# dtarb/TauDEM

Hardware: AMD Instinct MI355X
Metric: Mcells/s (PitRemove->D8FlowDir->AreaD8 pipeline) (higher is better)
Workload: dtype f32

## Files before the change

taudem_amd/csrc/flats.hpp:

```cpp
#pragma once
#include <algorithm>
#include <functional>
#include <vector>

#include "context.hpp"
#include "device_common.hpp"
#include "strips.hpp"
#include "tile_relax.hpp"

struct FlatLevels { int T; int Tr; int has_pits; };
struct FlatPhases { const char *classify, *levels, *stats, *directions, *next; };
static inline const FlatPhases& flat_phases(int iteration) {
    static const FlatPhases P[4] = {{"flats 1: classify", "flats 1: level fields", "flats 1: statistics", "flats 1: directions", "flats 1: next elev"},
                                    {"flats 2: classify", "flats 2: level fields", "flats 2: statistics", "flats 2: directions", "flats 2: next elev"},
                                    {"flats 3: classify", "flats 3: level fields", "flats 3: statistics", "flats 3: directions", "flats 3: next elev"},
                                    {"flats 4+: classify", "flats 4+: level fields", "flats 4+: statistics", "flats 4+: directions", "flats 4+: next elev"}};
    return P[iteration < 1 ? 0 : (iteration > 4 ? 3 : iteration - 1)];
}
using lvl_t = int16_t;
constexpr int LVL_SAT = 32767;
constexpr int TDX_FLATS_TOO_DEEP = -4242;
template <class LV>
struct FlatBuffersT { LV* lvl; LV* rq; };
using FlatBuffers = FlatBuffersT<lvl_t>;

template <class LV>
__host__ __device__ __forceinline__ LV flat_elev2(int lvl, int rq, FlatLevels fl) {
    const int e = (lvl < 0) ? 1 : (lvl > 0 ? lvl : 1 + fl.T);
    const int s = (rq > 0) ? (fl.Tr - rq + 1) : 0;
    return (LV)(e + s);
}

namespace flatk {
using namespace tdxk;

constexpr int CLASSIFY_ITEMS = 4;
template <class Traits, class LV>
__global__ __launch_bounds__(256) void classify_kernel(Traits tr, const float* __restrict__ Z, int nx, int tiles_x,
                                                       const uint32_t* __restrict__ list, unsigned long long nq, LV* __restrict__ lvl,
                                                       LV* __restrict__ rq, uint8_t* __restrict__ fmask, uint8_t* __restrict__ rmask,
                                                       uint32_t* __restrict__ tile_flags, uint8_t* __restrict__ tile_masked) {
    const unsigned long long base = (unsigned long long)blockIdx.x * (256 * CLASSIFY_ITEMS) + threadIdx.x;
#pragma unroll
    for (int i = 0; i < CLASSIFY_ITEMS; i++) {
        const unsigned long long q = base + (unsigned long long)i * 256;
        if (q < nq) {
            const size_t c = list[q];
            const float z0 = Z[c];
            bool low = false, quirk = false, higher = false;
            unsigned fm = 0, rm = 0;
#pragma unroll
            for (int k = 1; k <= 8; k++) {
                const size_t n = size_t(ptrdiff_t(c) + ptrdiff_t(d2(k)) * nx + d1(k));
                const float zd = z0 - Z[n];
                const bool inq = lvl[n] >= 0;
                if (zd < 0) higher = true;
                if (inq) rm |= 1u << (k - 1);
                if (!tr.dont_cross(c, nx, k)) {
                    if (zd >= 0 && tr.has_direction(n)) low = true;
                    else if (zd == 0) {
                        if (inq) fm |= 1u << (k - 1);
                        else quirk = true;
                    }
                }
            }
            if (low) lvl[c] = 1;
            else if (quirk) lvl[c] = 2;
            if (higher) rq[c] = 1;
            fmask[c] = uint8_t(low ? 0u : fm);
            rmask[c] = uint8_t(higher ? 0u : rm);
            const unsigned y = unsigned(c / size_t(nx)), x = unsigned(c - size_t(y) * size_t(nx));
            const unsigned tile = (y / tilek::TS) * unsigned(tiles_x) + x / tilek::TS;
            tile_flags[tile] = tilek::FLAG_FULL;
            if (!low && fm != rm) tile_masked[tile] = 1;
        }
    }
}

constexpr int CLS_COLS = 62, CLS_ROWS = 16;
template <class LV, class Src>
__global__ __launch_bounds__(256) void classify_stream_kernel(const float* __restrict__ Z, Src src, int nx, int ny,
                                                                 int y_own0, int y_own1, int tiles_x, LV* __restrict__ lvl,
                                                                 LV* __restrict__ rq, uint8_t* __restrict__ fmask, uint8_t* __restrict__ rmask,
                                                                 uint32_t* __restrict__ tile_flags, uint8_t* __restrict__ tile_masked, int nbx, int xmap,
                                                                 uint8_t* __restrict__ notfull) {
    using tilek::lane_left;
    using tilek::lane_right;
    const int bx = tdxk::xcd_block_x(nbx, xmap);
    if (bx < 0) return;
    const int lx = threadIdx.x & 63;
    const int x = bx * CLS_COLS - 1 + lx;
    const int ybase = __builtin_amdgcn_readfirstlane(y_own0 + blockIdx.y * (4 * CLS_ROWS) + (threadIdx.x >> 6) * CLS_ROWS);
    const bool mine = lx >= 1 && lx <= CLS_COLS && x < nx;
    const bool inx = x >= 0 && x < nx;
    const int xc = x < 0 ? 0 : (x >= nx ? nx - 1 : x);
    float z[CLS_ROWS + 2];
    typename Src::Raw pw[CLS_ROWS + 2];
#pragma unroll
    for (int j = 0; j < CLS_ROWS + 2; j++) {
        const int y = ybase - 1 + j, yc = y < 0 ? 0 : (y >= ny ? ny - 1 : y);
        const size_t o = size_t(yc) * size_t(nx) + size_t(xc);
        z[j] = Z[o];
        pw[j] = src.load(o);
    }
    unsigned ow[CLS_ROWS + 2];
#pragma unroll
    for (int j = 0; j < CLS_ROWS + 2; j++) {
        const int y = ybase - 1 + j;
        const bool in = inx && y >= 0 && y < ny;
        if (!in) z[j] = 0.f;
        ow[j] = in ? Src::onehot(pw[j]) : 0u;
    }
    int flag_row0 = -1, flag_row1 = -1;
    int masked_row = -1;
    unsigned fall_all = 0xFFu, rise_all = 0xFFu;
#pragma unroll
    for (int r = 0; r < CLS_ROWS; r++) {
        const int y = ybase + r;
        const float zn1 = z[r], zc1 = z[r + 1], zs1 = z[r + 2];
        const unsigned on1 = ow[r], oc1 = ow[r + 1], os1 = ow[r + 2];
        const float zn0 = lane_left(zn1, 0.f), zn2 = lane_right(zn1, 0.f), zc0 = lane_left(zc1, 0.f), zc2 = lane_right(zc1, 0.f);
        const float zs0 = lane_left(zs1, 0.f), zs2 = lane_right(zs1, 0.f);
        const unsigned on0 = lane_left(on1, 0u), on2 = lane_right(on1, 0u), oc0 = lane_left(oc1, 0u), oc2 = lane_right(oc1, 0u);
        const unsigned os0 = lane_left(os1, 0u), os2 = lane_right(os1, 0u);
        if (mine && y < y_own1) {
            const size_t idx = size_t(y) * size_t(nx) + size_t(x);
            LV l = -1, q = -1;
            unsigned fm = 0, rm = 0;
            if (oc1 & 1u) {
                const float z0 = zc1;
                bool higher = false;
                unsigned lowi = 0, fmq = 0;
#define TDX_CLS(K, ZN, ON, NC)                                                                                   \
    {                                                                                                             \
        const float zd = z0 - (ZN);                                                                               \
        const unsigned inq = (ON) & 1u, isdir = min((ON) & 0x1FEu, 1u), oth = ((ON) & 0x1FFu) ? 0u : 1u;          \
        higher |= zd < 0;                                                                                         \
        rm |= inq << ((K) - 1);                                                                                   \
        lowi |= zd >= 0 ? ((NC) & isdir) : 0u;                                                                    \
        fmq |= zd == 0 ? ((0u - (NC)) & ((inq << ((K) - 1)) | (oth << 8))) : 0u;                                  \
    }
                TDX_CLS(1, zc2, oc2, 1u)
                TDX_CLS(2, zn2, on2, (((oc2 >> 4) | (on1 >> 8)) & 1u) ^ 1u)
                TDX_CLS(3, zn1, on1, 1u)
                TDX_CLS(4, zn0, on0, (((on1 >> 6) | (oc0 >> 2)) & 1u) ^ 1u)
                TDX_CLS(5, zc0, oc0, 1u)
                TDX_CLS(6, zs0, os0, (((os1 >> 4) | (oc0 >> 8)) & 1u) ^ 1u)
                TDX_CLS(7, zs1, os1, 1u)
                TDX_CLS(8, zs2, os2, (((oc2 >> 6) | (os1 >> 2)) & 1u) ^ 1u)
#undef TDX_CLS
                const bool low = lowi != 0u, quirk = (fmq >> 8) != 0u;
                fm = fmq & 0xFFu;
                l = low ? 1 : (quirk ? 2 : 0);
                q = higher ? 1 : 0;
                const int tr = y / tilek::TS;
                if (!low && fm != rm) masked_row = tr;
                if (low) fm = 0;
                if (higher) rm = 0;
                if (flag_row0 < 0) flag_row0 = tr; else if (tr != flag_row0) flag_row1 = tr;
            }
            lvl[idx] = l;
            rq[idx] = q;
            fmask[idx] = uint8_t(fm);
            rmask[idx] = uint8_t(rm);
            fall_all &= fm;
            rise_all &= rm;
        }
    }
    if (notfull != nullptr && mine) {
        const int ylast = ybase + CLS_ROWS - 1;
        const int tr0 = ybase / tilek::TS, tr1 = (ylast < ny ? ylast : ny - 1) / tilek::TS;
        const bool short_seg = ylast >= y_own1;
        if (fall_all != 0xFFu || short_seg) { notfull[2 * (size_t(tr0) * tiles_x + x / tilek::TS)] = 1; if (tr1 != tr0) notfull[2 * (size_t(tr1) * tiles_x + x / tilek::TS)] = 1; }
        if (rise_all != 0xFFu || short_seg) { notfull[2 * (size_t(tr0) * tiles_x + x / tilek::TS) + 1] = 1; if (tr1 != tr0) notfull[2 * (size_t(tr1) * tiles_x + x / tilek::TS) + 1] = 1; }
    }
    if (flag_row0 >= 0) tile_flags[flag_row0 * tiles_x + x / tilek::TS] = tilek::FLAG_FULL;
    if (flag_row1 >= 0) tile_flags[flag_row1 * tiles_x + x / tilek::TS] = tilek::FLAG_FULL;
    if (masked_row >= 0) {
        tile_masked[flag_row0 * tiles_x + x / tilek::TS] = 1;
        if (flag_row1 >= 0) tile_masked[flag_row1 * tiles_x + x / tilek::TS] = 1;
    }
}

template <class S>
struct LevelPlainT {
    using T = int;
    static constexpr int kUniform = 8;
    S* G;
    const uint8_t* M;
    static __device__ __forceinline__ int inf() { return 0x3fffffff; }
    using Raw = S;
    using CellRaw = uint8_t;
    __device__ __forceinline__ S load_raw(size_t idx) const { return G[idx]; }
    static __device__ __forceinline__ int decode(S g) { return g > 0 ? int(g) : inf(); }
    static __device__ __forceinline__ bool raw_can_move(S g) { return g >= 0; }
    __device__ __forceinline__ void store(size_t idx, int v) const { G[idx] = S(sizeof(S) == 2 && v > LVL_SAT ? LVL_SAT : v); }
    __device__ __forceinline__ uint8_t cell_raw(size_t idx) const { return M[idx]; }
    static __device__ __forceinline__ void cell_decode(uint8_t m, int& lock, unsigned& mask) { lock = m ? 0 : inf(); mask = m; }
    static __device__ __forceinline__ int cell_floor(int lock, int v) { return lock == 0 ? 0 : v; }
    static __device__ __forceinline__ int apply(int lock, int own, int m) { return tilek::med3_raw(m + 1, lock, own); }
    static __device__ __forceinline__ bool settled(int, int v) { return v <= 1; }
    static __device__ __forceinline__ int act_never() { return int(0x80000000u); }
    static __device__ __forceinline__ int act_threshold(uint8_t m, int v) { return m ? v - 1 : act_never(); }
    static __device__ __forceinline__ int act_threshold_raw(S g) { return g >= 0 ? decode(g) - 1 : act_never(); }
};

constexpr int MACRO_KMAX = 8;
constexpr int MACRO_LMAX = MACRO_KMAX * 64 + 2;
constexpr int MACRO_INF = 0x3fffffff;
constexpr int MACRO_LDS_WORDS = 5 * MACRO_LMAX + 4 * (MACRO_LMAX - 2) + 8;

static __global__ __launch_bounds__(64) void find_blocks_kernel(const uint8_t* __restrict__ notfull, int tiles_x, int tiles_y, int nx, int y_lo, int y_hi, int kmax,
                                                                uint32_t* __restrict__ remapF, uint8_t* __restrict__ blkF, uint32_t* __restrict__ remapR, uint8_t* __restrict__ blkR) {
    const int field = int(blockIdx.y);
    uint32_t* const remap = field ? remapR : remapF;
    uint8_t* const blk_k = field ? blkR : blkF;
    const int rx = (tiles_x + 7) / 8;
    const int reg = blockIdx.x * 64 + threadIdx.x;
    if (reg >= rx * ((tiles_y + 7) / 8)) return;
    const int bx0 = (reg % rx) * 8, by0 = (reg / rx) * 8;
    unsigned long long fm = 0;
    const bool vec = (tiles_x & 7) == 0;
    for (int j = 0; j < 8; j++) {
        const int ty = by0 + j;
        if (ty >= tiles_y || ty * tilek::TS < y_lo || (ty + 1) * tilek::TS > y_hi) continue;
        unsigned rowbits = 0;
        if (vec) {
            const uint4 w = *reinterpret_cast<const uint4*>(notfull + 2 * (size_t(ty) * tiles_x + bx0));
            const unsigned ww[4] = {w.x, w.y, w.z, w.w};
#pragma unroll
            for (int i = 0; i < 8; i++) if (((ww[i >> 1] >> (16 * (i & 1) + 8 * field)) & 0xFFu) == 0u) rowbits |= 1u << i;
        } else {
            for (int i = 0; i < 8 && bx0 + i < tiles_x; i++) if (notfull[2 * (size_t(ty) * tiles_x + bx0 + i) + field] == 0) rowbits |= 1u << i;
        }
        for (int i = 0; i < 8; i++) if (bx0 + i >= tiles_x || (bx0 + i + 1) * tilek::TS > nx) rowbits &= ~(1u << i);
        fm |= (unsigned long long)rowbits << (8 * j);
    }
    auto full_block = [&](int i0, int j0, int kk) {
        unsigned long long m = 0;
        for (int b = 0; b < kk; b++) m |= ((kk == 8 ? 0xFFull : (kk == 4 ? 0xFull : 0x3ull)) << i0) << ((j0 + b) * 8);
        return (fm & m) == m;
    };
    for (int j = 0; j < 8; j++) {
        const int ty = by0 + j;
        if (ty >= tiles_y) break;
        for (int i = 0; i < 8; i++) {
            const int tx = bx0 + i;
            if (tx >= tiles_x) break;
            const size_t t = size_t(ty) * tiles_x + tx;
            int k = 0;
            for (int kk = kmax; kk >= 2 && !k; kk >>= 1) if (full_block(i & ~(kk - 1), j & ~(kk - 1), kk)) k = kk;
            if (k) {
                const int i0 = i & ~(k - 1), j0 = j & ~(k - 1);
                remap[t] = uint32_t(size_t(by0 + j0) * tiles_x + bx0 + i0) | (uint32_t(k == 8 ? 3 : (k == 4 ? 2 : 1)) << tilek::TILE_BLK_SHIFT);
                blk_k[t] = uint8_t((i == i0 && j == j0) ? k : 0);
            } else { remap[t] = uint32_t(t); blk_k[t] = 0; }
        }
    }
}

static __global__ __launch_bounds__(256) void block_flags_kernel(uint32_t* __restrict__ flags, const uint32_t* __restrict__ remap, int ntiles) {
    const int t = blockIdx.x * 256 + threadIdx.x;
    if (t < ntiles && tilek::entry_tile(remap[t]) != t) flags[t] = 0u;
}
__device__ __forceinline__ void macro_edge_scans(const int* __restrict__ h, int L, int* __restrict__ pre, int* __restrict__ suf, int* __restrict__ pm, int* __restrict__ sp) {
    const int wv = int(threadIdx.x >> 6), lane = int(threadIdx.x & 63);
    const bool fwd = (wv & 1) == 0;
    int* const out = wv == 0 ? pre : (wv == 1 ? suf : (wv == 2 ? pm : sp));
    int carry = MACRO_INF;
    for (int base = 0; base < L; base += 64) {
        const int j = fwd ? base + lane : L - 1 - base - lane;
        int v = MACRO_INF;
        if (j >= 0 && j < L) { v = h[j]; if (wv == 2) v -= j; else if (wv == 3) v += j; }
        {
#define TDX_MACRO_SCAN_STEP(CTRL, ROWS) { const int t = __builtin_amdgcn_update_dpp(MACRO_INF, v, CTRL, ROWS, 0xf, false); v = t < v ? t : v; }
            TDX_MACRO_SCAN_STEP(0x111, 0xf) TDX_MACRO_SCAN_STEP(0x112, 0xf) TDX_MACRO_SCAN_STEP(0x114, 0xf) TDX_MACRO_SCAN_STEP(0x118, 0xf)
            TDX_MACRO_SCAN_STEP(0x142, 0xa)
            TDX_MACRO_SCAN_STEP(0x143, 0xc)
#undef TDX_MACRO_SCAN_STEP
        }
        v = carry < v ? carry : v;
        if (j >= 0 && j < L) out[j] = v;
        carry = __shfl(v, 63, 64);
    }
}
__device__ __forceinline__ int macro_offer(const int* __restrict__ h, const int* __restrict__ pre, const int* __restrict__ suf, const int* __restrict__ pm,
                                           const int* __restrict__ sp, int L, int a, int d) {
    const int lo = a - d, hi = a + d;
    int near;
    if (lo <= 0) near = pre[hi < L - 1 ? hi : L - 1];
    else if (hi >= L - 1) near = suf[lo];
    else { near = h[lo]; for (int j = lo + 1; j <= hi; j++) near = h[j] < near ? h[j] : near; }
    int best = near + d;
    if (lo - 1 >= 0) { const int f = pm[lo - 1] + a; best = f < best ? f : best; }
    if (hi + 1 <= L - 1) { const int f = sp[hi + 1] - a; best = f < best ? f : best; }
    return best;
}

template <int INC, class S>
struct LevelOpT {
    using T = int;
    static constexpr int kMacroLdsWords = INC == 1 ? MACRO_LDS_WORDS : 0;
    static constexpr int kUniform = 0;
    S* G;
    const uint8_t* M;
    const uint8_t* TM = nullptr;
    static constexpr bool kHasPlain = INC == 1;
    using Plain = LevelPlainT<S>;
    __device__ __forceinline__ Plain plain() const { return Plain{G, M}; }
    __device__ __forceinline__ bool tile_masked(int tile) const { return TM != nullptr && TM[tile] != 0; }
    static __device__ __forceinline__ int inf() { return 0x3fffffff; }
    using Raw = S;
    using CellRaw = uint8_t;
    __device__ __forceinline__ S load_raw(size_t idx) const { return G[idx]; }
    static __device__ __forceinline__ int decode(S g) { return g > 0 ? int(g) : inf(); }
    static __device__ __forceinline__ bool raw_can_move(S g) { return g >= 0; }
    __device__ __forceinline__ void store(size_t idx, int v) const { G[idx] = S(v); }
    __device__ __forceinline__ uint8_t cell_raw(size_t idx) const { return M[idx]; }
    static __device__ __forceinline__ void cell_decode(uint8_t m, int& cst, unsigned& mask) { cst = 0; mask = m; }
    static __device__ __forceinline__ int apply(int, int own, int m) {
        int t = m + INC;
        if (sizeof(S) == 2 && INC) t = unsigned(t - LVL_SAT) < unsigned(inf() - LVL_SAT) ? LVL_SAT : t;
        return t < own ? t : own;
    }
    static __device__ __forceinline__ int cell_floor(int cst, int) { return cst; }
    static __device__ __forceinline__ bool settled(int, int v) { return v <= 1; }
    static __device__ __forceinline__ int act_never() { return int(0x80000000u); }
    static __device__ __forceinline__ int act_threshold(uint8_t m, int v) { return m ? v - INC : act_never(); }
    static __device__ __forceinline__ int act_threshold_raw(S g) { return g >= 0 ? decode(g) - INC : act_never(); }

    __device__ __forceinline__ int macro_update(const tilek::TileGeom& g, int tile, int k, int* __restrict__ lds, tilek::TileLds& TL, uint32_t* __restrict__ flags_next,
                                                unsigned long long* __restrict__ dbg = nullptr) const {
        const int tid = int(threadIdx.x);
        const unsigned long long tq0 = dbg ? __builtin_readcyclecounter() : 0ull;
        const int W = k * tilek::TS, L = W + 2;
        const int tx0 = tile % g.tiles_x, ty0 = tile / g.tiles_x;
        const int X0 = tx0 * tilek::TS, Y0 = ty0 * tilek::TS;
        const size_t pitch = size_t(g.nx);
        int* const h = lds; int* const pre = h + MACRO_LMAX; int* const suf = pre + MACRO_LMAX; int* const pm = suf + MACRO_LMAX; int* const sp = pm + MACRO_LMAX;
        int* const acc = sp + MACRO_LMAX;
        int* const moved = acc + 4 * (MACRO_LMAX - 2);
        constexpr int AW = MACRO_LMAX - 2;
        if (tid < 8) moved[tid] = 0;
        __syncthreads();
        auto rim_idx = [&](int e, int i) -> size_t {
            const int x = e == 2 ? 0 : (e == 3 ? W - 1 : i), y = e == 0 ? 0 : (e == 1 ? W - 1 : i);
            return size_t(Y0 + y) * pitch + size_t(X0 + x);
        };
        S raw_rim[4][2], raw_ring[4][3];
        unsigned ring_ok = 0;
        int out_target = -1;
        if (tid < 4 * (k + 2)) {
            const int e = tid / (k + 2), j = tid % (k + 2) - 1;
            const int ntx = e == 2 ? tx0 - 1 : (e == 3 ? tx0 + k : tx0 + j), nty = e == 0 ? ty0 - 1 : (e == 1 ? ty0 + k : ty0 + j);
            if (ntx >= 0 && ntx < g.tiles_x && nty >= 0 && nty < g.tiles_y) out_target = int(g.remap[size_t(nty) * g.tiles_x + ntx]);
        }
#pragma unroll
        for (int e = 0; e < 4; e++)
#pragma unroll
            for (int u = 0; u < 2; u++) {
                const int i = tid + u * 256;
                raw_rim[e][u] = G[rim_idx(e, i < W ? i : W - 1)];
// ... 410 lines not shown
    if (nq_old) hipLaunchKernelGGL((flatk::unmark_q_kernel<LV>), dim3(tdx_blocks_for(nq_old, 256)), dim3(256), 0, ctx->stream, qold, nq_old, lvl, rq);
    if (nq) hipLaunchKernelGGL((flatk::reset_q_kernel<LV>), dim3(tdx_blocks_for(nq, 256)), dim3(256), 0, ctx->stream, qlist, nq, lvl, rq);
    int rc = strip_exchange<LV>(ctx, st, lvl, LV(-1));
    if (rc != TDX_OK) return rc;
    return strip_exchange<LV>(ctx, st, rq, LV(-1));
}

template <class LV>
static inline int flats_overwrite_elevation_sparse(tdx_context* ctx, int nx, const uint32_t* qlist, unsigned long long nq, const LV* lvl, const LV* rq,
                                                   FlatLevels fl, float* zout) {
    TdxSpan sp(ctx, TDX_K_MISC);
    if (nq) hipLaunchKernelGGL((flatk::overwrite_elev_sparse_kernel<LV>), dim3(tdx_blocks_for(nq, 256)), dim3(256), 0, ctx->stream, qlist, nq, nx, lvl, rq, fl, zout);
    return TDX_OK;
}

template <class LV>
static inline int flats_overwrite_elevation(tdx_context* ctx, size_t n, const LV* lvl, const LV* rq, FlatLevels fl, float* zout) {
    TdxSpan sp(ctx, TDX_K_MISC);
    hipLaunchKernelGGL((flatk::overwrite_elev_kernel<LV>), dim3(tdx_blocks_for(n, 256)), dim3(256), 0, ctx->stream, n, lvl, rq, fl, zout);
    return TDX_OK;
}

template <class Op = flatk::LevelOp>
static inline int flats_relax_field(tdx_context* ctx, const Strip& st, tilek::TileGeom geom, typename Op::Raw* field, const uint8_t* mask, tilek::Sched sc,
                                    int64_t* rounds, int64_t* launches, const uint8_t* tile_masked = nullptr, int eager_rounds = 0) {
    Op op{field, mask};
    if constexpr (Op::kHasPlain) op.TM = tile_masked;
    for (;;) {
        bool left = false;
        int rc = (st.multi() && eager_rounds > 0) ? tile_relax_run_bounded(ctx, op, geom, sc, eager_rounds, &left, rounds, launches) : tile_relax_run(ctx, op, geom, sc, rounds, launches);
        if (rc != TDX_OK) return rc;
        if (!st.multi()) return TDX_OK;
        int64_t changed = 0;
        rc = strip_exchange<typename Op::Raw>(ctx, st, field, typename Op::Raw(-1), sc.flags, geom.tiles_x, &changed, true, left ? 1 : 0);
        if (rc != TDX_OK) return rc;
        if (changed == 0) return TDX_OK;
    }
}

using StreamClassifyFn = std::function<void(const tilek::TileGeom&, uint8_t* fmask, uint8_t* rmask, uint32_t* tile_flags, uint8_t* tile_masked, uint8_t* notfull)>;
template <class Traits, class LV>
static int flats_bfs(tdx_context* ctx, Traits tr, const float* Z, const Strip& st, const uint32_t* qlist, unsigned long long nq,
                     FlatBuffersT<LV> b, FlatLevels* out, tdx_stats* stats, const StreamClassifyFn* stream_classify = nullptr, int iteration = 1) {
    using LOp = flatk::LevelOpT<1, LV>;
    const FlatPhases& ph = flat_phases(iteration);
    ctx->phase = ph.classify;
    hipStream_t s = ctx->stream;
    const int nx = st.nx;
    const size_t n = size_t(nx) * size_t(st.ny_arr);
    const tilek::TileGeom geom = tilek::make_geom(nx, st.ny_arr, st.y0, st.y1);
    const int ntiles = geom.tiles_x * geom.tiles_y;
    unsigned long long* d_cnt = reinterpret_cast<unsigned long long*>(ctx->d_mail);
    uint8_t* fmask = static_cast<uint8_t*>(ctx->scratch(TDX_S_E, n));
    uint8_t* rmask = static_cast<uint8_t*>(ctx->scratch(TDX_S_F, n));
    uint32_t* flags0 = static_cast<uint32_t*>(ctx->scratch(TDX_S_G, size_t(ntiles) * 4 * 2 + size_t(ntiles)));
    uint32_t* list = static_cast<uint32_t*>(ctx->scratch(TDX_S_H, size_t(ntiles) * 4 * tilek::SCHED_LIST_WORDS));
    unsigned long long* counts = static_cast<unsigned long long*>(ctx->scratch(TDX_S_K, size_t(tilek::COUNT_RING) * 16));
    if (!fmask || !rmask || !flags0 || !list || !counts) return TDX_ERR_NOMEM;
    uint32_t* flags = flags0 + ntiles;
    uint8_t* tmask = reinterpret_cast<uint8_t*>(flags0 + 2 * size_t(ntiles));
    const char* e_masked = getenv("TDX_FLATS_MASKED");
    const bool no_plain = e_masked && e_masked[0] == '1';
    const bool half_plain = e_masked && e_masked[0] == '2';
    TdxSpan sp(ctx, TDX_K_BFS);
    static const bool no_pair = getenv("TDX_FLATS_SEQUENTIAL") != nullptr;
    static const bool strips_sequential = getenv("TDX_FLATS_STRIPS_SEQUENTIAL") != nullptr;
    const bool pair = !(st.multi() && strips_sequential) && !ctx->kernel_timing && !no_pair;
    uint32_t* flagsB = pair ? static_cast<uint32_t*>(ctx->scratch(TDX_S_L, size_t(ntiles) * 4 * (1 + tilek::SCHED_LIST_WORDS))) : nullptr;
    unsigned long long* countsB = pair ? static_cast<unsigned long long*>(ctx->scratch(TDX_S_M, size_t(tilek::COUNT_RING) * 16)) : nullptr;
    if (pair && (!flagsB || !countsB)) return TDX_ERR_NOMEM;
    int macro_k = 0;
    if constexpr (sizeof(LV) == 2) {
        const char* e_macro = getenv("TDX_FLATS_MACRO");
        macro_k = e_macro ? atoi(e_macro) : flatk::MACRO_KMAX;
        macro_k = macro_k >= 8 ? 8 : (macro_k >= 4 ? 4 : (macro_k >= 2 ? 2 : 0));
        if (!stream_classify || getenv("TDX_FLATS_FUSED") != nullptr || getenv("TDX_RELAX_LDS") != nullptr || no_plain || half_plain) macro_k = 0;
    }
    uint8_t* notfull = nullptr; uint32_t *remapF = nullptr, *remapR = nullptr, *fill_list = nullptr; uint8_t *blkF = nullptr, *blkR = nullptr;
    if (macro_k) {
        uint8_t* m = static_cast<uint8_t*>(ctx->scratch(TDX_S_MACRO, size_t(ntiles) * 20 + 64));
        if (!m) return TDX_ERR_NOMEM;
        notfull = m; blkF = m + 2 * size_t(ntiles); blkR = blkF + ntiles;
        remapF = reinterpret_cast<uint32_t*>(m + 4 * size_t(ntiles)); remapR = remapF + ntiles; fill_list = remapR + ntiles;
    }
    hipLaunchKernelGGL(flatk::prepare_kernel, dim3(tdx_blocks_for(size_t(std::max(ntiles, 2 * tilek::COUNT_RING)), 256)), dim3(256), 0, s, d_cnt, flags0, tmask, ntiles,
                       no_plain ? 1 : (half_plain ? 2 : 0), counts, countsB, notfull);
    if (stream_classify) (*stream_classify)(geom, fmask, rmask, flags0, tmask, notfull);
    else {
        const bool clear_masks = getenv("TDX_RELAX_LDS") != nullptr || getenv("TDX_RELAX_ASYNC") != nullptr || getenv("TDX_FLATS_CLEAR_MASKS") != nullptr;
        if (clear_masks) {
            TDX_HIP_CHECK(ctx, hipMemsetAsync(fmask, 0, n, s));
            TDX_HIP_CHECK(ctx, hipMemsetAsync(rmask, 0, n, s));
        }
        if (nq)
            hipLaunchKernelGGL((flatk::classify_kernel<Traits, LV>), dim3(tdx_blocks_for(nq, 256 * flatk::CLASSIFY_ITEMS)), dim3(256), 0, s, tr, Z, nx,
                               geom.tiles_x, qlist, nq, b.lvl, b.rq, fmask, rmask, flags0, tmask);
    }
    int rc = strip_exchange<LV>(ctx, st, b.lvl, LV(-1));
    if (rc != TDX_OK) return rc;
    ctx->phase = ph.levels;
    rc = strip_exchange<LV>(ctx, st, b.rq, LV(-1));
    if (rc != TDX_OK) return rc;
    int64_t launches = 1, rounds_fall = 0, rounds_rise = 0;
    tilek::TileGeom geomF = geom, geomR = geom;
    if (macro_k) {
        const int y_lo = st.multi() ? st.y0 + 1 : st.y0, y_hi = st.multi() ? st.y1 - 1 : st.y1;
        const unsigned nreg = unsigned(((geom.tiles_x + 7) / 8) * ((geom.tiles_y + 7) / 8));
        hipLaunchKernelGGL(flatk::find_blocks_kernel, dim3((nreg + 63) / 64, 2), dim3(64), 0, s, notfull, geom.tiles_x, geom.tiles_y, nx, y_lo, y_hi, macro_k, remapF, blkF, remapR, blkR);
        geomF.remap = remapF; geomF.blk_k = blkF;
        geomR.remap = remapR; geomR.blk_k = blkR;
    }
    if (pair) {
        uint32_t* listB = flagsB + ntiles;
        const bool two_streams = getenv("TDX_FLATS_FUSED") == nullptr || getenv("TDX_RELAX_LDS") != nullptr;
        const uint32_t* start_flags = two_streams ? flags0 : nullptr;
        if (!two_streams) {
            TDX_HIP_CHECK(ctx, hipMemcpyAsync(flags, flags0, size_t(ntiles) * 4, hipMemcpyDeviceToDevice, s));
            TDX_HIP_CHECK(ctx, hipMemcpyAsync(flagsB, flags0, size_t(ntiles) * 4, hipMemcpyDeviceToDevice, s));
        }
        for (;;) {
            rc = two_streams ? tile_relax_run_pair(ctx, LOp{b.lvl, fmask, tmask}, tilek::Sched{flags, list, counts},
                                                   LOp{b.rq, rmask, no_plain ? tmask : nullptr}, tilek::Sched{flagsB, listB, countsB}, geomF, &rounds_fall, &launches, start_flags, &geomR)
                             : tile_relax_run_fused(ctx, LOp{b.lvl, fmask, tmask}, tilek::Sched{flags, list, counts},
                                                    LOp{b.rq, rmask, no_plain ? tmask : nullptr}, tilek::Sched{flagsB, listB, countsB}, geom, &rounds_fall, &launches);
            if (rc != TDX_OK) return rc;
            start_flags = nullptr;
            if (!st.multi()) break;
            int64_t ch_fall = 0, ch_rise = 0;
            rc = strip_exchange<LV>(ctx, st, b.lvl, LV(-1), flags, geom.tiles_x, &ch_fall);
            if (rc != TDX_OK) return rc;
            rc = strip_exchange<LV>(ctx, st, b.rq, LV(-1), flagsB, geom.tiles_x, &ch_rise);
            if (rc != TDX_OK) return rc;
            int64_t changed = ch_fall + ch_rise;
            rc = strip_allreduce(ctx, st, &changed, 1, TDX_OP_SUM);
            if (rc != TDX_OK) return rc;
            if (changed == 0) break;
        }
    } else {
        const unsigned cg = tdx_blocks_for(size_t(ntiles), 256);
        TDX_HIP_CHECK(ctx, hipMemcpyAsync(flags, flags0, size_t(ntiles) * 4, hipMemcpyDeviceToDevice, s));
        if (macro_k) hipLaunchKernelGGL(flatk::block_flags_kernel, dim3(cg), dim3(256), 0, s, flags, remapF, ntiles);
        rc = flats_relax_field<LOp>(ctx, st, geomF, b.lvl, fmask, tilek::Sched{flags, list, counts}, &rounds_fall, &launches, tmask);
// ... 60 lines not shown
```

taudem_amd/csrc/tile_relax.hpp:

```cpp
#pragma once
#include <atomic>
#include <algorithm>
#include <chrono>
#include <cstdlib>
#include <functional>
#include <type_traits>

#include "context.hpp"
#include "device_common.hpp"

namespace tilek {
using namespace tdxk;

constexpr int TS = 64;
constexpr int LH = TS + 2;
constexpr int LP = LH + 1;
constexpr int RPW = 16;
constexpr int NWAVE = TS / RPW;
constexpr int NTHR = NWAVE * 64;
constexpr int COUNT_RING = 1024;
constexpr int MAX_SWEEPS = 8;
constexpr int PULL_MAX = 64;
constexpr unsigned MACRO_DEAL_MAX = 4096;
constexpr unsigned MACRO_WGS_MIN = MACRO_DEAL_MAX / PULL_MAX;

struct TileGeom {
    int nx, ny;
    int tiles_x, tiles_y;
    int y_own0, y_own1;
    int max_sweeps;
    int chain_max;
    unsigned long long* cnt_host;
    const unsigned long long* cnt_dev;
    unsigned long long cnt_tag;
    int act_filter;
    const uint32_t* remap;
    const uint8_t* blk_k;
};

static inline TileGeom make_geom(int nx, int ny, int y_own0, int y_own1) {
    TileGeom g;
    g.nx = nx; g.ny = ny;
    g.tiles_x = (nx + TS - 1) / TS; g.tiles_y = (ny + TS - 1) / TS;
    g.y_own0 = y_own0; g.y_own1 = y_own1;
    static const int ms = getenv("TDX_MAX_SWEEPS") ? atoi(getenv("TDX_MAX_SWEEPS")) : MAX_SWEEPS;
    g.max_sweeps = ms;
    static const int cm = getenv("TDX_SOLO_CHAIN") ? atoi(getenv("TDX_SOLO_CHAIN")) : 256;
    g.chain_max = cm;
    g.cnt_host = nullptr; g.cnt_dev = nullptr; g.cnt_tag = 0ull;
    static const int af = getenv("TDX_ACT_FILTER_OFF") ? 0 : 1;
    g.act_filter = af;
    g.remap = nullptr; g.blk_k = nullptr;
    return g;
}

template <class T>
__device__ __forceinline__ T masked_min(unsigned mask, T inf, T e, T ne, T n, T nw, T w, T sw, T s, T se) {
    T m = inf;
    if (mask & 1u) m = e < m ? e : m;
    if (mask & 2u) m = ne < m ? ne : m;
    if (mask & 4u) m = n < m ? n : m;
    if (mask & 8u) m = nw < m ? nw : m;
    if (mask & 16u) m = w < m ? w : m;
    if (mask & 32u) m = sw < m ? sw : m;
    if (mask & 64u) m = s < m ? s : m;
    if (mask & 128u) m = se < m ? se : m;
    return m;
}

template <class T>
__device__ __forceinline__ T uniform_min(bool fourway, T e, T ne, T n, T nw, T w, T sw, T s, T se) {
    T m = e < n ? e : n;
    const T m2 = w < s ? w : s;
    m = m2 < m ? m2 : m;
    if (!fourway) {
        T d = ne < nw ? ne : nw;
        const T d2 = sw < se ? sw : se;
        d = d2 < d ? d2 : d;
        m = d < m ? d : m;
    }
    return m;
}


__device__ __forceinline__ unsigned mask_at(const unsigned (&pk)[RPW / 4], int r) { return (pk[r >> 2] >> (8 * (r & 3))) & 0xFFu; }

struct TileLds {
    int rim;
    unsigned long long top[2][NWAVE], bot[2][NWAVE];
    unsigned any[2][NWAVE];
    unsigned rows[NWAVE];
    unsigned next;
    unsigned long long base;
    unsigned npend;
    int chain;
    uint32_t pulled[PULL_MAX];
    uint32_t pend[PULL_MAX * 9];
};

constexpr uint32_t FLAG_HALO = 1u, FLAG_FULL = 2u;
constexpr uint32_t TILE_IDX_MASK = 0x07ffffffu;
constexpr int TILE_BLK_SHIFT = 27;
__device__ __forceinline__ int entry_tile(uint32_t e) { return int(e & TILE_IDX_MASK); }
__device__ __forceinline__ int entry_blk_k(uint32_t e) { const unsigned c = (e >> TILE_BLK_SHIFT) & 3u; return c ? 1 << c : 0; }
// ... 327 lines not shown
    s.ra = lane_right(a, s.ra);
    s.lb = lane_left(b, s.lb);
    s.rb = lane_right(b, s.rb);
    if (Op::kUniform == 8) return min3_raw(min3_raw(a, s.la, s.ra), min3_raw(s.lc, s.rc, b), min3_raw(s.lb, s.rb, hm));
    const T inf = Op::inf();
    return min3_raw(min3_raw(keep_if_bit(m8, 0, s.rc, inf), keep_if_bit(m8, 1, s.ra, inf), keep_if_bit(m8, 2, a, inf)),
                    min3_raw(keep_if_bit(m8, 3, s.la, inf), keep_if_bit(m8, 4, s.lc, inf), keep_if_bit(m8, 5, s.lb, inf)),
                    min3_raw(keep_if_bit(m8, 6, b, inf), keep_if_bit(m8, 7, s.rb, inf), hm));
}
template <class Op>
__device__ __forceinline__ typename Op::T halo_min(unsigned m8, bool left, bool right, typename Op::T ha, typename Op::T hc, typename Op::T hb) {
    using T = typename Op::T;
    const T inf = Op::inf();
    if (!left && !right) return inf;
    if (Op::kUniform == 4) return hc;
    if (Op::kUniform == 8) return min3_raw(ha, hc, hb);
    return left ? min3_raw(keep_if_bit(m8, 3, ha, inf), keep_if_bit(m8, 4, hc, inf), keep_if_bit(m8, 5, hb, inf))
                : min3_raw(keep_if_bit(m8, 1, ha, inf), keep_if_bit(m8, 0, hc, inf), keep_if_bit(m8, 7, hb, inf));
}

template <class T>
__device__ __forceinline__ unsigned shift_in_ne(unsigned x, T a, T b) {
    static_assert(sizeof(T) == 4, "32-bit values");
    if constexpr (std::is_same<T, float>::value)
        asm("v_cmp_neq_f32 vcc, %1, %2\n\tv_addc_co_u32 %0, vcc, %0, %0, vcc" : "+v"(x) : "v"(a), "v"(b) : "vcc");
    else
        asm("v_cmp_ne_u32 vcc, %1, %2\n\tv_addc_co_u32 %0, vcc, %0, %0, vcc" : "+v"(x) : "v"(a), "v"(b) : "vcc");
    return x;
}

__device__ __forceinline__ unsigned wave_or(unsigned x) {
    int y = int(x);
    y |= __builtin_amdgcn_update_dpp(0, y, 0x111, 0xf, 0xf, true);
    y |= __builtin_amdgcn_update_dpp(0, y, 0x112, 0xf, 0xf, true);
    y |= __builtin_amdgcn_update_dpp(0, y, 0x114, 0xf, 0xf, true);
    y |= __builtin_amdgcn_update_dpp(0, y, 0x118, 0xf, 0xf, true);
    return unsigned(__builtin_amdgcn_readlane(y, 15) | __builtin_amdgcn_readlane(y, 31) | __builtin_amdgcn_readlane(y, 47) | __builtin_amdgcn_readlane(y, 63));
}

template <class Op, class = void>
struct has_act_threshold : std::false_type {};
template <class Op>
struct has_act_threshold<Op, std::void_t<decltype(Op::act_never())>> : std::true_type {};
template <class Op, class = void>
struct has_act_threshold_raw : std::false_type {};
template <class Op>
struct has_act_threshold_raw<Op, std::void_t<decltype(Op::act_threshold_raw(typename Op::Raw()))>> : std::true_type {};
template <class T>
__device__ __forceinline__ T max_t(T a, T b) { return a > b ? a : b; }
template <class Op, class = void>
struct has_raw_can_move : std::false_type {};
template <class Op>
struct has_raw_can_move<Op, std::void_t<decltype(Op::raw_can_move(typename Op::Raw()))>> : std::true_type {};

template <class Op>
__device__ __forceinline__ int relax_tile_reg(const Op& op, const TileGeom& g, int tile, typename Op::T* sV, TileLds& L, unsigned long long* __restrict__ dbg) {
    using T = typename Op::T;
    const int tid = threadIdx.x;
    const int lx = tid & 63;
    const int wv = tid >> 6;
    const int ry0 = wv * RPW;
    const int tx = tile % g.tiles_x, ty = tile / g.tiles_x;
    const int x0 = tx * TS, y0 = ty * TS;
    T* sSide = sV;
    T* sRow = sV + 2 * LH;
    const unsigned long long tc0 = dbg ? __builtin_readcyclecounter() : 0ull;
    if (tid == 0) L.rim = 0;
    if (lx == 0) L.rows[wv] = 0u;
    const int gx = x0 + lx;
    const bool col_ok = gx < g.nx;
    const int gxc = col_ok ? gx : g.nx - 1;
    const long long row_pitch = (long long)g.nx;
    typename Op::Raw raw[RPW], raw_edge, raw_side;
    typename Op::CellRaw craw[RPW], craw_edge = {};
    {
        int gy = y0 + ry0;
#pragma unroll
        for (int r = 0; r < RPW; r++) {
            const int gyc = gy >= g.ny ? g.ny - 1 : gy;
            const size_t idx = size_t((long long)gyc * row_pitch + gxc);
            raw[r] = op.load_raw(idx);
            craw[r] = op.cell_raw(idx);
            gy++;
        }
    }
    const int ey = (wv == 0) ? y0 - 1 : y0 + TS;
    const bool edge_ok = col_ok && ey >= 0 && ey < g.ny;
    bool side_ok;
    {
        const int eyc = ey < 0 ? 0 : (ey >= g.ny ? g.ny - 1 : ey);
        raw_edge = op.load_raw(size_t((long long)eyc * row_pitch + gxc));
        if constexpr (has_act_threshold<Op>::value && !has_act_threshold_raw<Op>::value) craw_edge = op.cell_raw(size_t((long long)eyc * row_pitch + gxc));
        const int row = (tid >> 1) < LH ? (tid >> 1) : LH - 1, right = tid & 1;
        const int sx = right ? x0 + TS : x0 - 1, sy = y0 - 1 + row;
        side_ok = tid < 2 * LH && sx >= 0 && sx < g.nx && sy >= 0 && sy < g.ny;
        const int sxc = sx < 0 ? 0 : (sx >= g.nx ? g.nx - 1 : sx), syc = sy < 0 ? 0 : (sy >= g.ny ? g.ny - 1 : sy);
        raw_side = op.load_raw(size_t((long long)syc * row_pitch + sxc));
    }
    T v[RPW], cst[RPW];
    unsigned mk[RPW / 4] = {};
    unsigned live = 0;
#pragma unroll
    for (int r = 0; r < RPW; r++) {
        const int gy = y0 + ry0 + r;
        v[r] = (col_ok && gy < g.ny) ? Op::decode(raw[r]) : Op::inf();
        T c = Op::inf();
        unsigned m = 0;
        bool movable = col_ok && gy >= g.y_own0 && gy < g.y_own1;
        if constexpr (has_raw_can_move<Op>::value) movable = movable && Op::raw_can_move(raw[r]);
        if (movable) Op::cell_decode(craw[r], c, m);
        if (m && !Op::settled(c, v[r])) live |= 1u << r;
        cst[r] = Op::cell_floor(c, v[r]);
        mk[r >> 2] |= (m & 0xFFu) << (8 * (r & 3));
    }
    const T edge_row = edge_ok ? Op::decode(raw_edge) : Op::inf();
    if (tid < 2 * LH) sSide[(tid & 1) * LH + (tid >> 1)] = side_ok ? Op::decode(raw_side) : Op::inf();
    T* sEdgeT = sRow + 2 * NWAVE * 2 * TS;
    T* sSideT = sEdgeT + 2 * TS;
    if constexpr (has_act_threshold<Op>::value) {
        T te;
        if constexpr (has_act_threshold_raw<Op>::value) te = edge_ok ? Op::act_threshold_raw(raw_edge) : Op::act_never();
        else te = edge_ok ? Op::act_threshold(craw_edge, Op::decode(raw_edge)) : Op::act_never();
        const T te3 = max_t(te, max_t(lane_left(te, Op::act_never()), lane_right(te, Op::act_never())));
        if (wv == 0) sEdgeT[lx] = te3;
        if (wv == NWAVE - 1) sEdgeT[TS + lx] = te3;
        if constexpr (has_act_threshold_raw<Op>::value)
            if (tid < 2 * LH) sSideT[(tid & 1) * LH + (tid >> 1)] = side_ok ? Op::act_threshold_raw(raw_side) : Op::act_never();
    }
    sRow[((0 * NWAVE + wv) * 2 + 0) * TS + lx] = v[0];
    sRow[((0 * NWAVE + wv) * 2 + 1) * TS + lx] = v[RPW - 1];
    if (live) atomicOr(&L.rows[wv], live);
    __syncthreads();
    T hm[RPW];
    {
        const bool left = lx == 0, right = lx == TS - 1;
        T sd[RPW + 2];
#pragma unroll
        for (int j = 0; j < RPW + 2; j++) sd[j] = sSide[(right ? LH : 0) + ry0 + j];
#pragma unroll
        for (int r = 0; r < RPW; r++) hm[r] = halo_min<Op>(mask_at(mk, r), left, right, sd[r], sd[r + 1], sd[r + 2]);
    }
    ShiftRegs<T> sh = {Op::inf(), Op::inf(), Op::inf(), Op::inf(), Op::inf(), Op::inf()};
    const unsigned rows_live = __builtin_amdgcn_readfirstlane(L.rows[wv]);
    unsigned moved = 0;
    const unsigned long long tc1 = dbg ? __builtin_readcyclecounter() : 0ull;
    bool any_change = false, capped = false;
    unsigned rows = rows_live;
    for (int iter = 0;; iter++) {
        const int cur = iter & 1;
        const T up = (wv == 0) ? edge_row : sRow[((cur * NWAVE + wv - 1) * 2 + 1) * TS + lx];
        const T dn = (wv == NWAVE - 1) ? edge_row : sRow[((cur * NWAVE + wv + 1) * 2 + 0) * TS + lx];
        unsigned chg_lane = 0;
        if (rows == 0u) {
        } else if ((iter & 1) == 0) {
#pragma unroll
            for (int r = 0; r < RPW; r++) {
                const T a = r ? v[r ? r - 1 : 0] : up, c = v[r], b = (r < RPW - 1) ? v[r < RPW - 1 ? r + 1 : r] : dn;
                unsigned m8 = mask_at(mk, r);
                if (Op::kUniform == 0) asm volatile("" : "+v"(m8));
                const T m = reg_row_min<Op>(m8, a, c, b, hm[r], sh);
                const T wn = Op::apply(cst[r], c, m);
                chg_lane = shift_in_ne(chg_lane, wn, c);
                v[r] = wn;
            }
            chg_lane = __builtin_bitreverse32(chg_lane) >> (32 - RPW);
        } else {
#pragma unroll
            for (int r = RPW - 1; r >= 0; r--) {
                const T a = r ? v[r ? r - 1 : 0] : up, c = v[r], b = (r < RPW - 1) ? v[r < RPW - 1 ? r + 1 : r] : dn;
                unsigned m8 = mask_at(mk, r);
                if (Op::kUniform == 0) asm volatile("" : "+v"(m8));
                const T m = reg_row_min<Op>(m8, a, c, b, hm[r], sh);
                const T wn = Op::apply(cst[r], c, m);
                chg_lane = shift_in_ne(chg_lane, wn, c);
                v[r] = wn;
            }
        }
        moved |= chg_lane;
        const unsigned chg_rows = wave_or(chg_lane);
        sRow[(((cur ^ 1) * NWAVE + wv) * 2 + 0) * TS + lx] = v[0];
        sRow[(((cur ^ 1) * NWAVE + wv) * 2 + 1) * TS + lx] = v[RPW - 1];
        if (lx == 0) {
            L.any[cur][wv] = chg_rows != 0u;
            L.top[cur][wv] = chg_rows & 1u;
            L.bot[cur][wv] = (chg_rows >> (RPW - 1)) & 1u;
        }
        __syncthreads();
        unsigned any = 0;
#pragma unroll
        for (int w = 0; w < NWAVE; w++) any |= L.any[cur][w];
        if (any) any_change = true;
        if (!any || iter + 1 >= g.max_sweeps) {
            capped = any != 0;
            if (dbg && tid == 0) { atomicAdd(dbg, (unsigned long long)(iter + 1)); atomicAdd(dbg + 1, 1ull); }
            break;
        }
        unsigned nd = (chg_rows | (chg_rows << 1) | (chg_rows >> 1)) & ((1u << RPW) - 1u);
        const unsigned above = wv > 0 ? unsigned(L.bot[cur][wv > 0 ? wv - 1 : 0]) : 0u, below = wv < NWAVE - 1 ? unsigned(L.top[cur][wv < NWAVE - 1 ? wv + 1 : 0]) : 0u;
        if (above) nd |= 1u;
        if (below) nd |= 1u << (RPW - 1);
        rows = __builtin_amdgcn_readfirstlane(nd) & rows_live;
    }
    const unsigned long long tc2 = dbg ? __builtin_readcyclecounter() : 0ull;
    if (any_change) {
        int rim = 0;
#pragma unroll
        for (int r = 0; r < RPW; r++) {
            const int ly = ry0 + r;
            if ((moved >> r) & 1u) {
                op.store(size_t(y0 + ly) * size_t(g.nx) + size_t(gx), v[r]);
                const bool top = (ly == 0), bot = (ly == TS - 1), lef = (lx == 0), rig = (lx == TS - 1);
                if constexpr (has_act_threshold<Op>::value) {
                    const bool all = g.act_filter == 0;
                    if ((top || bot) && (all || v[r] < sEdgeT[(bot ? TS : 0) + lx])) rim |= top ? 1 : 2;
                    if constexpr (has_act_threshold_raw<Op>::value) {
                        if (lef || rig) {
                            const T* st = sSideT + (rig ? LH : 0);
                            if (all || v[r] < max_t(st[ly], max_t(st[ly + 1], st[ly + 2]))) rim |= lef ? 4 : 8;
                            if (top && (all || v[r] < st[0])) rim |= lef ? 16 : 32;
                            if (bot && (all || v[r] < st[LH - 1])) rim |= lef ? 64 : 128;
                        }
                    } else {
                        if (lef) rim |= 4;
                        if (rig) rim |= 8;
                        if (top && lef) rim |= 16;
                        if (top && rig) rim |= 32;
                        if (bot && lef) rim |= 64;
                        if (bot && rig) rim |= 128;
                    }
                } else {
                    if (top) rim |= 1;
                    if (bot) rim |= 2;
                    if (lef) rim |= 4;
                    if (rig) rim |= 8;
                    if (top && lef) rim |= 16;
                    if (top && rig) rim |= 32;
                    if (bot && lef) rim |= 64;
                    if (bot && rig) rim |= 128;
                }
            }
        }
        if (rim) atomicOr(&L.rim, rim);
    }
    __syncthreads();
    if (dbg && tid == 0) {
        const unsigned long long tc3 = __builtin_readcyclecounter();
        atomicAdd(dbg + 6, tc1 - tc0); atomicAdd(dbg + 7, tc2 - tc1); atomicAdd(dbg + 8, tc3 - tc2);
    }
    const int res = (any_change ? (L.rim | RES_CHANGED) : 0) | (capped ? RES_CAPPED : 0);
    __syncthreads();
    return res;
}

__device__ __forceinline__ int activation_target(int res, int tile, const TileGeom& g, uint32_t* flag) {
    const int tid = threadIdx.x;
    int target = -1;
    *flag = FLAG_HALO;
    if (tid < 8 && ((res >> tid) & 1)) {
        const int ddx[8] = {0, 0, -1, 1, -1, 1, -1, 1};
        const int ddy[8] = {-1, 1, 0, 0, -1, -1, 1, 1};
        const int tx = tile % g.tiles_x, ty = tile / g.tiles_x;
        const int ntx = tx + ddx[tid], nty = ty + ddy[tid];
        if (ntx >= 0 && ntx < g.tiles_x && nty >= 0 && nty < g.tiles_y) target = nty * g.tiles_x + ntx;
        if (g.remap != nullptr && target >= 0) target = int(g.remap[target]);
    }
    if (tid == 8 && (res & RES_CAPPED)) { target = tile; *flag = FLAG_FULL; }
    return target;
}
__device__ __forceinline__ void flag_neighbours(int res, int tile, const TileGeom& g, uint32_t* __restrict__ flags_next, TileLds& L) {
    uint32_t flag;
    const int target = activation_target(res, tile, g, &flag);
    if (target >= 0 && atomicMax(&flags_next[entry_tile(uint32_t(target))], flag) == 0u) L.pend[atomicAdd(&L.npend, 1u)] = uint32_t(target);
}
template <class Body>
__device__ __forceinline__ void round_driver(const uint32_t* __restrict__ list, unsigned long long* __restrict__ count, uint32_t* __restrict__ flags_cur,
                                             uint32_t* __restrict__ flags_next, uint32_t* __restrict__ list_next, unsigned pull_max, const TileGeom& g,
                                             TileLds& L, Body body, unsigned bid, unsigned nblocks) {
    const int chain_max = g.chain_max;
    const unsigned nact = unsigned(count[0]);
    if (g.cnt_host != nullptr && bid == 0u && threadIdx.x == 0)
        __hip_atomic_store(g.cnt_host + (count - g.cnt_dev), g.cnt_tag | (unsigned long long)count[0], __ATOMIC_RELAXED, __HIP_MEMORY_SCOPE_SYSTEM);
    const uint32_t entry0 = list[bid];
    unsigned long long* cursor = count + COUNT_RING;
    unsigned pull = nact / (2u * nblocks);
    pull = pull < 1u ? 1u : (pull > pull_max ? pull_max : pull);
    const bool fixed = nact <= nblocks;
    if (bid * pull >= nact) return;
    if (threadIdx.x == 0) L.npend = 0u;
    for (unsigned turn = 0;; turn++) {
        __syncthreads();
        const unsigned npend = L.npend;
        if (threadIdx.x == 0) {
            L.base = npend ? atomicAdd(count + 1, (unsigned long long)npend) : 0ull;
            L.next = fixed ? (turn == 0u ? bid : nact) : unsigned(atomicAdd(cursor, (unsigned long long)pull));
        }
// ... 762 lines not shown
```

Baseline: 13450.

## Drop rise-mask buffer from plain flats path and ballot-reduce tile rim flags

The plain level-relaxation operator no longer reads a per-cell mask array; it assumes every cell is unlocked with all eight neighbours enabled. As a result the rmask buffer is only allocated and written when the masked or clear-mask modes are requested, which saves a byte per cell of global writes in classify and a load per cell in relaxation. The tile write-back now computes rim activation flags with wave ballots and an LDS column staging step instead of per-thread branching, at the cost of an extra __syncthreads. The new assumption about the plain path only holds if that operator is only used on tiles without masking.

After: 13900 (median of 6 runs). 1.03x the previous value.

```diff
diff --git a/taudem_amd/csrc/flats.hpp b/taudem_amd/csrc/flats.hpp
--- a/taudem_amd/csrc/flats.hpp
+++ b/taudem_amd/csrc/flats.hpp
@@ -68,7 +68,7 @@
             else if (quirk) lvl[c] = 2;
             if (higher) rq[c] = 1;
             fmask[c] = uint8_t(low ? 0u : fm);
-            rmask[c] = uint8_t(higher ? 0u : rm);
+            if (rmask != nullptr) rmask[c] = uint8_t(higher ? 0u : rm);
             const unsigned y = unsigned(c / size_t(nx)), x = unsigned(c - size_t(y) * size_t(nx));
             const unsigned tile = (y / tilek::TS) * unsigned(tiles_x) + x / tilek::TS;
             tile_flags[tile] = tilek::FLAG_FULL;
@@ -162,7 +162,7 @@
             lvl[idx] = l;
             rq[idx] = q;
             fmask[idx] = uint8_t(fm);
-            rmask[idx] = uint8_t(rm);
+            if (rmask != nullptr) rmask[idx] = uint8_t(rm);
             fall_all &= fm;
             rise_all &= rm;
         }
@@ -187,21 +187,17 @@
     using T = int;
     static constexpr int kUniform = 8;
     S* G;
-    const uint8_t* M;
     static __device__ __forceinline__ int inf() { return 0x3fffffff; }
     using Raw = S;
-    using CellRaw = uint8_t;
     __device__ __forceinline__ S load_raw(size_t idx) const { return G[idx]; }
     static __device__ __forceinline__ int decode(S g) { return g > 0 ? int(g) : inf(); }
     static __device__ __forceinline__ bool raw_can_move(S g) { return g >= 0; }
     __device__ __forceinline__ void store(size_t idx, int v) const { G[idx] = S(sizeof(S) == 2 && v > LVL_SAT ? LVL_SAT : v); }
-    __device__ __forceinline__ uint8_t cell_raw(size_t idx) const { return M[idx]; }
-    static __device__ __forceinline__ void cell_decode(uint8_t m, int& lock, unsigned& mask) { lock = m ? 0 : inf(); mask = m; }
+    static __device__ __forceinline__ void cell_decode(int& lock, unsigned& mask) { lock = 0; mask = 0xFFu; }
     static __device__ __forceinline__ int cell_floor(int lock, int v) { return lock == 0 ? 0 : v; }
     static __device__ __forceinline__ int apply(int lock, int own, int m) { return tilek::med3_raw(m + 1, lock, own); }
     static __device__ __forceinline__ bool settled(int, int v) { return v <= 1; }
     static __device__ __forceinline__ int act_never() { return int(0x80000000u); }
-    static __device__ __forceinline__ int act_threshold(uint8_t m, int v) { return m ? v - 1 : act_never(); }
     static __device__ __forceinline__ int act_threshold_raw(S g) { return g >= 0 ? decode(g) - 1 : act_never(); }
 };
 
@@ -307,7 +303,7 @@
     const uint8_t* TM = nullptr;
     static constexpr bool kHasPlain = INC == 1;
     using Plain = LevelPlainT<S>;
-    __device__ __forceinline__ Plain plain() const { return Plain{G, M}; }
+    __device__ __forceinline__ Plain plain() const { return Plain{G}; }
     __device__ __forceinline__ bool tile_masked(int tile) const { return TM != nullptr && TM[tile] != 0; }
     static __device__ __forceinline__ int inf() { return 0x3fffffff; }
     using Raw = S;
@@ -824,16 +820,18 @@
     const int ntiles = geom.tiles_x * geom.tiles_y;
     unsigned long long* d_cnt = reinterpret_cast<unsigned long long*>(ctx->d_mail);
     uint8_t* fmask = static_cast<uint8_t*>(ctx->scratch(TDX_S_E, n));
-    uint8_t* rmask = static_cast<uint8_t*>(ctx->scratch(TDX_S_F, n));
     uint32_t* flags0 = static_cast<uint32_t*>(ctx->scratch(TDX_S_G, size_t(ntiles) * 4 * 2 + size_t(ntiles)));
     uint32_t* list = static_cast<uint32_t*>(ctx->scratch(TDX_S_H, size_t(ntiles) * 4 * tilek::SCHED_LIST_WORDS));
     unsigned long long* counts = static_cast<unsigned long long*>(ctx->scratch(TDX_S_K, size_t(tilek::COUNT_RING) * 16));
-    if (!fmask || !rmask || !flags0 || !list || !counts) return TDX_ERR_NOMEM;
+    if (!fmask || !flags0 || !list || !counts) return TDX_ERR_NOMEM;
     uint32_t* flags = flags0 + ntiles;
     uint8_t* tmask = reinterpret_cast<uint8_t*>(flags0 + 2 * size_t(ntiles));
     const char* e_masked = getenv("TDX_FLATS_MASKED");
     const bool no_plain = e_masked && e_masked[0] == '1';
     const bool half_plain = e_masked && e_masked[0] == '2';
+    const bool clear_masks = getenv("TDX_RELAX_LDS") != nullptr || getenv("TDX_RELAX_ASYNC") != nullptr || getenv("TDX_FLATS_CLEAR_MASKS") != nullptr;
+    uint8_t* rmask = (no_plain || clear_masks) ? static_cast<uint8_t*>(ctx->scratch(TDX_S_F, n)) : nullptr;
+    if ((no_plain || clear_masks) && !rmask) return TDX_ERR_NOMEM;
     TdxSpan sp(ctx, TDX_K_BFS);
     static const bool no_pair = getenv("TDX_FLATS_SEQUENTIAL") != nullptr;
     static const bool strips_sequential = getenv("TDX_FLATS_STRIPS_SEQUENTIAL") != nullptr;
@@ -859,7 +857,6 @@
                        no_plain ? 1 : (half_plain ? 2 : 0), counts, countsB, notfull);
     if (stream_classify) (*stream_classify)(geom, fmask, rmask, flags0, tmask, notfull);
     else {
-        const bool clear_masks = getenv("TDX_RELAX_LDS") != nullptr || getenv("TDX_RELAX_ASYNC") != nullptr || getenv("TDX_FLATS_CLEAR_MASKS") != nullptr;
         if (clear_masks) {
             TDX_HIP_CHECK(ctx, hipMemsetAsync(fmask, 0, n, s));
             TDX_HIP_CHECK(ctx, hipMemsetAsync(rmask, 0, n, s));
diff --git a/taudem_amd/csrc/tile_relax.hpp b/taudem_amd/csrc/tile_relax.hpp
--- a/taudem_amd/csrc/tile_relax.hpp
+++ b/taudem_amd/csrc/tile_relax.hpp
@@ -48,8 +48,7 @@
     static const int cm = getenv("TDX_SOLO_CHAIN") ? atoi(getenv("TDX_SOLO_CHAIN")) : 256;
     g.chain_max = cm;
     g.cnt_host = nullptr; g.cnt_dev = nullptr; g.cnt_tag = 0ull;
-    static const int af = getenv("TDX_ACT_FILTER_OFF") ? 0 : 1;
-    g.act_filter = af;
+    g.act_filter = getenv("TDX_ACT_FILTER_OFF") ? 0 : 1;
     g.remap = nullptr; g.blk_k = nullptr;
     return g;
 }
@@ -483,6 +482,11 @@
 struct has_raw_can_move : std::false_type {};
 template <class Op>
 struct has_raw_can_move<Op, std::void_t<decltype(Op::raw_can_move(typename Op::Raw()))>> : std::true_type {};
+struct NoCellRaw {};
+template <class Op, class = void>
+struct cell_raw_of { using type = NoCellRaw; static constexpr bool value = false; };
+template <class Op>
+struct cell_raw_of<Op, std::void_t<typename Op::CellRaw>> { using type = typename Op::CellRaw; static constexpr bool value = true; };
 
 template <class Op>
 __device__ __forceinline__ int relax_tile_reg(const Op& op, const TileGeom& g, int tile, typename Op::T* sV, TileLds& L, unsigned long long* __restrict__ dbg) {
@@ -503,7 +507,8 @@
     const int gxc = col_ok ? gx : g.nx - 1;
     const long long row_pitch = (long long)g.nx;
     typename Op::Raw raw[RPW], raw_edge, raw_side;
-    typename Op::CellRaw craw[RPW], craw_edge = {};
+    constexpr bool kCellRaw = cell_raw_of<Op>::value;
+    typename cell_raw_of<Op>::type craw[RPW], craw_edge = {};
     {
         int gy = y0 + ry0;
 #pragma unroll
@@ -511,7 +516,7 @@
             const int gyc = gy >= g.ny ? g.ny - 1 : gy;
             const size_t idx = size_t((long long)gyc * row_pitch + gxc);
             raw[r] = op.load_raw(idx);
-            craw[r] = op.cell_raw(idx);
+            if constexpr (kCellRaw) craw[r] = op.cell_raw(idx);
             gy++;
         }
     }
@@ -539,7 +544,10 @@
         unsigned m = 0;
         bool movable = col_ok && gy >= g.y_own0 && gy < g.y_own1;
         if constexpr (has_raw_can_move<Op>::value) movable = movable && Op::raw_can_move(raw[r]);
-        if (movable) Op::cell_decode(craw[r], c, m);
+        if (movable) {
+            if constexpr (kCellRaw) Op::cell_decode(craw[r], c, m);
+            else Op::cell_decode(c, m);
+        }
         if (m && !Op::settled(c, v[r])) live |= 1u << r;
         cst[r] = Op::cell_floor(c, v[r]);
         mk[r >> 2] |= (m & 0xFFu) << (8 * (r & 3));
@@ -634,34 +642,51 @@
     }
     const unsigned long long tc2 = dbg ? __builtin_readcyclecounter() : 0ull;
     if (any_change) {
-        int rim = 0;
-#pragma unroll
-        for (int r = 0; r < RPW; r++) {
-            const int ly = ry0 + r;
-            if ((moved >> r) & 1u) {
-                op.store(size_t(y0 + ly) * size_t(g.nx) + size_t(gx), v[r]);
-                const bool top = (ly == 0), bot = (ly == TS - 1), lef = (lx == 0), rig = (lx == TS - 1);
-                if constexpr (has_act_threshold<Op>::value) {
-                    const bool all = g.act_filter == 0;
-                    if ((top || bot) && (all || v[r] < sEdgeT[(bot ? TS : 0) + lx])) rim |= top ? 1 : 2;
-                    if constexpr (has_act_threshold_raw<Op>::value) {
-                        if (lef || rig) {
-                            const T* st = sSideT + (rig ? LH : 0);
-                            if (all || v[r] < max_t(st[ly], max_t(st[ly + 1], st[ly + 2]))) rim |= lef ? 4 : 8;
-                            if (top && (all || v[r] < st[0])) rim |= lef ? 16 : 32;
-                            if (bot && (all || v[r] < st[LH - 1])) rim |= lef ? 64 : 128;
-                        }
+        if constexpr (has_act_threshold_raw<Op>::value) {
+            int rim = 0;
+            const int wvu = __builtin_amdgcn_readfirstlane(wv);
+            const bool all = g.act_filter == 0;
+            if (wvu == 0 && __ballot((moved & 1u) != 0u && (all || v[0] < sEdgeT[lx])) != 0ull) rim |= 1;
+            if (wvu == NWAVE - 1 && __ballot(((moved >> (RPW - 1)) & 1u) != 0u && (all || v[RPW - 1] < sEdgeT[TS + lx])) != 0ull) rim |= 2;
+            T* sCol = sRow;
+            if (lx == 0 || lx == TS - 1) {
+                T* col = sCol + (lx ? TS : 0) + ry0;
+#pragma unroll
+                for (int r = 0; r < RPW; r++) col[r] = ((moved >> r) & 1u) ? v[r] : Op::inf();
+            }
+            __syncthreads();
+            size_t idx = size_t(y0 + ry0) * size_t(g.nx) + size_t(gx);
+#pragma unroll
+            for (int r = 0; r < RPW; r++) {
+                if ((moved >> r) & 1u) op.store(idx, v[r]);
+                idx += size_t(g.nx);
+            }
+            if (wvu < 2) {
+                const T val = sCol[wvu * TS + lx];
+                const T* st = sSideT + wvu * LH;
+                const bool mv = val < Op::inf();
+                const bool side = all ? mv : val < max_t(st[lx], max_t(st[lx + 1], st[lx + 2]));
+                const bool c_top = lx == 0 && (all ? mv : val < st[0]);
+                const bool c_bot = lx == TS - 1 && (all ? mv : val < st[LH - 1]);
+                if (__ballot(side) != 0ull) rim |= 4 << wvu;
+                if (__ballot(c_top) != 0ull) rim |= 16 << wvu;
+                if (__ballot(c_bot) != 0ull) rim |= 64 << wvu;
+            }
+            if (rim && lx == 0) atomicOr(&L.rim, rim);
+        } else {
+            int rim = 0;
+#pragma unroll
+            for (int r = 0; r < RPW; r++) {
+                const int ly = ry0 + r;
+                if ((moved >> r) & 1u) {
+                    op.store(size_t(y0 + ly) * size_t(g.nx) + size_t(gx), v[r]);
+                    const bool top = (ly == 0), bot = (ly == TS - 1), lef = (lx == 0), rig = (lx == TS - 1);
+                    if constexpr (has_act_threshold<Op>::value) {
+                        if ((top || bot) && (g.act_filter == 0 || v[r] < sEdgeT[(bot ? TS : 0) + lx])) rim |= top ? 1 : 2;
                     } else {
-                        if (lef) rim |= 4;
-                        if (rig) rim |= 8;
-                        if (top && lef) rim |= 16;
-                        if (top && rig) rim |= 32;
-                        if (bot && lef) rim |= 64;
-                        if (bot && rig) rim |= 128;
+                        if (top) rim |= 1;
+                        if (bot) rim |= 2;
                     }
-                } else {
-                    if (top) rim |= 1;
-                    if (bot) rim |= 2;
                     if (lef) rim |= 4;
                     if (rig) rim |= 8;
                     if (top && lef) rim |= 16;
@@ -670,8 +695,8 @@
                     if (bot && rig) rim |= 128;
                 }
             }
-        }
-        if (rim) atomicOr(&L.rim, rim);
+            if (rim) atomicOr(&L.rim, rim);
+        }
     }
     __syncthreads();
     if (dbg && tid == 0) {
```
